# shenyunhang/APE

Hardware: NVIDIA H100
Metric: images_per_sec (higher is better)
Workload: dtype f16

## Files before the change

### ape_b200/csrc/gemm_tc.cu

```cuda
#include <stdlib.h>

#include <type_traits>

#include "common.cuh"
#include "tc.cuh"

namespace ape {
namespace {

constexpr int BM = 128, BK = 64, WG_K = 16;
constexpr int kConsumerWarps = 8;
constexpr int kThreads = 32 * kConsumerWarps + 32;

enum Act { ACT_NONE = 0, ACT_RELU = 1, ACT_GELU = 2, ACT_SWIGLU = 3, ACT_CLAMP = 4 };
enum Res { RES_NONE = 0, RES_F32 = 1, RES_16 = 2 };

template <bool OUT32, int ACT, int RES, bool LN = false, bool ROPE = false, bool STATS = false>
struct Epi {
  static constexpr bool out32 = OUT32, ln = LN, rope = ROPE, stats = STATS;
  static constexpr int act = ACT, res = RES;
};

struct GemmParams {
  void *C;
  const float *bias;
  const void *residual;
  long long ldc, ldr;
  int M, N, K;
  int m_blocks, n_blocks, k_blocks;
  int band;
  int vec_out;
  int fast;
  const float *rope_cos, *rope_sin;
  const int *rope_pos;
  int rope_cols, rope_npos;
  const float *ln_part;
  const float *ln_colsum;
  int ln_nparts;
  float ln_inv_c, ln_eps;
  float *stats_out;
  int stats_nslab;
  int conv;
  int conv_tw, conv_th, conv_tiles_x, conv_tiles_img, conv_cblks, conv_W, conv_H;
  long long *trace;
  int argmax_col_base;
};

__device__ __forceinline__ void trace_stamp(const GemmParams &p, int slot) {
  if (p.trace != nullptr) p.trace[(size_t)blockIdx.x * 8 + slot] = clock64();
}

template <int BN, int STAGES>
struct alignas(1024) GemmSmem {
  uint8_t a[STAGES][BM * BK * 2];
  uint8_t b[STAGES][BN * BK * 2];
  uint64_t full[STAGES], empty[STAGES];
};

template <int ACT>
__device__ __forceinline__ float act1(float v) {
  if constexpr (ACT == ACT_RELU) return fmaxf(v, 0.f);
  if constexpr (ACT == ACT_GELU) return 0.5f * v * (1.f + erff(v * 0.70710678118654752f));
  if constexpr (ACT == ACT_CLAMP) return fminf(fmaxf(v, -50000.f), 50000.f);
  return v;
}

template <bool VEC>
__device__ __forceinline__ float2 ld_pair(const float *p, int n, bool ok1) {
  if constexpr (VEC) return __ldg(reinterpret_cast<const float2 *>(p + n));
  return make_float2(__ldg(p + n), ok1 ? __ldg(p + n + 1) : 0.f);
}
template <bool VEC, typename T>
__device__ __forceinline__ float2 ld_res_pair(const T *p, bool ok1) {
  if constexpr (VEC) return Elem<T>::load2(p);
  return make_float2(Elem<T>::load1(p), ok1 ? Elem<T>::load1(p + 1) : 0.f);
}

__device__ __forceinline__ size_t out_row_offset(const GemmParams &p, int m) {
  if (!p.conv) return (size_t)m * p.ldc;
  const int m_blk = m / BM, r = m - m_blk * BM;
  const int img = m_blk / p.conv_tiles_img, t = m_blk - img * p.conv_tiles_img;
  const int ty = t / p.conv_tiles_x, tx = t - ty * p.conv_tiles_x;
  const int x = tx * p.conv_tw + r % p.conv_tw, y = ty * p.conv_th + r / p.conv_tw;
  return (((size_t)img * p.conv_H + y) * p.conv_W + x) * p.ldc;
}

template <typename TO>
__device__ __forceinline__ void store_pair(TO *dst, float v0, float v1, bool ok1, bool vec) {
  if (vec && ok1) {
    if constexpr (sizeof(TO) == 4) {
      *reinterpret_cast<float2 *>(dst) = make_float2(v0, v1);
    } else if constexpr (std::is_same<TO, __half>::value) {
      *reinterpret_cast<__half2 *>(dst) = __floats2half2_rn(v0, v1);
    } else {
      *reinterpret_cast<__nv_bfloat162 *>(dst) = __floats2bfloat162_rn(v0, v1);
    }
  } else {
    dst[0] = Elem<TO>::from_f(v0);
    if (ok1) dst[1] = Elem<TO>::from_f(v1);
  }
}

template <class E, typename TI, int BN, bool FULL>
__device__ __forceinline__ void epilogue(const GemmParams &p, const float *acc, int m_blk, int n_blk, int wg, int lane) {
  using TO = std::conditional_t<E::out32, float, TI>;
  constexpr bool swiglu = E::act == ACT_SWIGLU;
  const int warp4 = (threadIdx.x >> 5) & 3, tq = lane & 3;
  const int c_base = n_blk * BN + 2 * tq;
  TO *C = reinterpret_cast<TO *>(p.C);
#pragma unroll
  for (int h = 0; h < 2; ++h) {
    const int m = m_blk * BM + wg * 64 + warp4 * 16 + (lane >> 2) + 8 * h;
    const bool row_ok = FULL || m < p.M;
    const int mr = row_ok ? m : p.M - 1;
    float ln_rstd = 1.f, ln_shift = 0.f;
    if constexpr (E::ln) {
      const float2 *pp = reinterpret_cast<const float2 *>(p.ln_part) + (size_t)mr * p.ln_nparts;
      float sum = 0.f, sq = 0.f;
      for (int i = 0; i < p.ln_nparts; ++i) {
        const float2 t = __ldg(pp + i);
        sum += t.x;
        sq += t.y;
      }
      const float mean = sum * p.ln_inv_c;
      ln_rstd = rsqrtf(fmaxf(sq * p.ln_inv_c - mean * mean, 0.f) + p.ln_eps);
      ln_shift = ln_rstd * mean;
    }
    int rope_row = 0;
    if constexpr (E::rope) rope_row = (p.rope_pos ? __ldg(p.rope_pos + mr) : mr % p.rope_npos) * 64;
    TO *crow = C + out_row_offset(p, mr);
    const float *res32 = reinterpret_cast<const float *>(p.residual) + (size_t)mr * p.ldr;
    const TI *res16 = reinterpret_cast<const TI *>(p.residual) + (size_t)mr * p.ldr;
    float st_sum = 0.f, st_sq = 0.f;
#pragma unroll
    for (int j = 0; j < BN / 8; ++j) {
      const int n = c_base + 8 * j;
      const bool ok0 = FULL || n < p.N, ok1 = FULL || n + 1 < p.N;
      float v0 = acc[4 * j + 2 * h], v1 = acc[4 * j + 2 * h + 1];
      if (ok0) {
        if constexpr (E::ln) {
          const float2 cs = ld_pair<FULL>(p.ln_colsum, n, ok1);
          v0 = fmaf(ln_rstd, v0, -ln_shift * cs.x);
          if (ok1) v1 = fmaf(ln_rstd, v1, -ln_shift * cs.y);
        }
        if (p.bias != nullptr) {
          const float2 b = ld_pair<FULL && !E::ln>(p.bias, n, ok1);
          v0 += b.x;
          if (ok1) v1 += b.y;
        }
      }
      if constexpr (swiglu) {
        const float o = v0 / (1.f + __expf(-v0)) * v1;
        const TO ot = Elem<TO>::from_f(o);
        if (ok0 && row_ok) crow[n / 2] = ot;
        if constexpr (E::stats) {
          const float f = ok0 ? Elem<TO>::to_f(ot) : 0.f;
          st_sum += f;
          st_sq = fmaf(f, f, st_sq);
          if ((j & 15) == 15) {
            st_sum += __shfl_xor_sync(0xffffffffu, st_sum, 1);
            st_sq += __shfl_xor_sync(0xffffffffu, st_sq, 1);
            st_sum += __shfl_xor_sync(0xffffffffu, st_sum, 2);
            st_sq += __shfl_xor_sync(0xffffffffu, st_sq, 2);
            const int slab_idx = (n_blk * BN + 8 * (j - 15)) / 128;
            if (tq == 0 && row_ok && slab_idx < p.stats_nslab)
              *reinterpret_cast<float2 *>(p.stats_out + ((size_t)m * p.stats_nslab + slab_idx) * 2) = make_float2(st_sum, st_sq);
            st_sum = 0.f;
            st_sq = 0.f;
          }
        }
        continue;
      } else {
        if constexpr (E::rope) {
          if (n < p.rope_cols) {
            const float2 c = __ldg(reinterpret_cast<const float2 *>(p.rope_cos + rope_row + (n & 63)));
            const float2 s = __ldg(reinterpret_cast<const float2 *>(p.rope_sin + rope_row + (n & 63)));
            const float t0 = v0, t1 = v1;
            v0 = t0 * c.x - t1 * s.x;
            v1 = t1 * c.y + t0 * s.y;
          }
        }
        v0 = act1<E::act>(v0);
        v1 = act1<E::act>(v1);
        if constexpr (E::res != RES_NONE) {
          if (ok0) {
            const float2 r = E::res == RES_F32 ? ld_res_pair<FULL>(res32 + n, ok1) : ld_res_pair<FULL>(res16 + n, ok1);
            v0 += r.x;
            if (ok1) v1 += r.y;
          }
        }
        if (ok0 && row_ok) store_pair<TO>(crow + n, v0, v1, ok1, FULL || p.vec_out);
      }
    }
  }
}

struct EpiArgmax {
  static constexpr bool out32 = true, ln = false, rope = false, stats = false;
  static constexpr int act = ACT_NONE, res = RES_NONE;
};
template <class E>
constexpr bool kArgmax = std::is_same<E, EpiArgmax>::value;

template <int BN>
__device__ __forceinline__ void argmax_epilogue(const GemmParams &p, const float *acc, int m_blk, int n_blk, int wg, int lane) {
  const int warp4 = (threadIdx.x >> 5) & 3, tq = lane & 3;
  const int c_base = n_blk * BN + 2 * tq;
  unsigned long long *keys = reinterpret_cast<unsigned long long *>(p.C);
#pragma unroll
  for (int h = 0; h < 2; ++h) {
    const int m = m_blk * BM + wg * 64 + warp4 * 16 + (lane >> 2) + 8 * h;
    float best = -INFINITY;
    int col = -1;
#pragma unroll
    for (int j = 0; j < BN / 8; ++j) {
      const int n = c_base + 8 * j;
      const float v0 = acc[4 * j + 2 * h], v1 = acc[4 * j + 2 * h + 1];
      if (n < p.N && (col < 0 || v0 > best)) { best = v0; col = n; }
      if (n + 1 < p.N && v1 > best) { best = v1; col = n + 1; }
    }
#pragma unroll
    for (int s = 1; s <= 2; s <<= 1) {
      const float ob = __shfl_xor_sync(0xffffffffu, best, s);
      const int oc = __shfl_xor_sync(0xffffffffu, col, s);
      if (oc >= 0 && (col < 0 || ob > best || (ob == best && oc < col))) { best = ob; col = oc; }
    }
    if (tq == 0 && col >= 0 && m < p.M) atomicMax(keys + m, argmax_key(best, col + p.argmax_col_base));
  }
}

template <int BN, int STAGES, int CL, typename TI, class E>
__global__ void __launch_bounds__(kThreads, 1)
gemm_tc_kernel(const __grid_constant__ CUtensorMap map_a, const __grid_constant__ CUtensorMap map_b, const GemmParams p) {
  extern __shared__ uint8_t smem_raw[];
  pdl_launch_dependents();
  if (threadIdx.x == 0) trace_stamp(p, 0);
  using Smem = GemmSmem<BN, STAGES>;
  Smem &s = *reinterpret_cast<Smem *>((reinterpret_cast<uintptr_t>(smem_raw) + 1023) & ~uintptr_t(1023));
  constexpr uint32_t STAGE_BYTES = (BM + BN) * BK * 2;

  const int warp = threadIdx.x / 32, lane = threadIdx.x % 32;
  const int rank = CL > 1 ? (int)tc::cluster_ctarank() : 0;
  const int m_groups = (p.m_blocks + CL - 1) / CL;
  const int num_tiles = m_groups * p.n_blocks;
  const int first = blockIdx.x / CL, stride = gridDim.x / CL;
  auto tile_at = [&](int t, int &m_blk, int &n_blk) -> bool {
    const int tile = first + t * stride;
    if (tile >= num_tiles) return false;
    const int per_band = p.band * p.n_blocks;
    const int band = tile / per_band, r = tile - band * per_band;
    const int rows = min(p.band, m_groups - band * p.band);
    n_blk = r / rows;
    m_blk = (band * p.band + r - n_blk * rows) * CL + rank;
    return true;
  };

  if (warp == kConsumerWarps && lane == 0) {
    tc::prefetch_tensormap(&map_a);
    tc::prefetch_tensormap(&map_b);
#pragma unroll
    for (int i = 0; i < STAGES; ++i) {
      tc::mbar_init(&s.full[i], 1);
      tc::mbar_init(&s.empty[i], kConsumerWarps * CL);
    }
    tc::fence_mbar_init();
  }
  __syncthreads();
  if (CL > 1) tc::cluster_sync_all();
  pdl_wait();
  if (threadIdx.x == 0) trace_stamp(p, 1);

  if (warp == kConsumerWarps) {
    if (lane == 0) {
      uint32_t stage = 0, phase = 0;
      int m_blk, n_blk;
      for (int t = 0; tile_at(t, m_blk, n_blk); ++t) {
        for (int kb = 0; kb < p.k_blocks; ++kb) {
          tc::mbar_wait(&s.empty[stage], phase ^ 1);
          tc::mbar_expect_tx(&s.full[stage], STAGE_BYTES);
          if (p.conv) {
            const int img = m_blk / p.conv_tiles_img, tt = m_blk - img * p.conv_tiles_img;
            const int ty = tt / p.conv_tiles_x, tx = tt - ty * p.conv_tiles_x;
            const int tap = kb / p.conv_cblks, cb = kb - tap * p.conv_cblks;
            tc::tma_load_4d(s.a[stage], &map_a, &s.full[stage], cb * BK, tx * p.conv_tw + tap % 3 - 1, ty * p.conv_th + tap / 3 - 1, img);
          } else {
            tc::tma_load_2d(s.a[stage], &map_a, &s.full[stage], kb * BK, m_blk * BM);
          }
          if (CL == 1) {
            tc::tma_load_2d(s.b[stage], &map_b, &s.full[stage], kb * BK, n_blk * BN);
          } else {
            constexpr int HALF_ROWS = BN / CL;
            tc::tma_load_2d_multicast(s.b[stage] + rank * HALF_ROWS * BK * 2, &map_b, &s.full[stage], kb * BK,
                                      n_blk * BN + rank * HALF_ROWS, (uint16_t)((1u << CL) - 1));
          }
          if (++stage == STAGES) { stage = 0; phase ^= 1; }
        }
      }
    }
    __syncwarp();
  } else {
    const int wg = warp / 4;
    float acc[BN / 2];
#pragma unroll
    for (int i = 0; i < BN / 2; ++i) acc[i] = 0.f;
    auto release = [&](uint32_t st) {
      if (lane == 0) {
        tc::mbar_arrive(&s.empty[st]);
        if (CL > 1) tc::mbar_arrive_cluster(tc::mapa_u32(&s.empty[st], (uint32_t)(rank ^ 1)));
      }
    };
    uint32_t stage = 0, phase = 0;
    int m_blk, n_blk;
    for (int t = 0; tile_at(t, m_blk, n_blk); ++t) {
      uint32_t prev = 0;
      for (int kb = 0; kb < p.k_blocks; ++kb) {
        tc::mbar_wait(&s.full[stage], phase);
        if (kb == 0 && t == 0 && threadIdx.x == 0) trace_stamp(p, 2);
        const uint64_t da = tc::make_smem_desc_sw128(tc::smem_u32(s.a[stage] + wg * 64 * BK * 2));
        const uint64_t db = tc::make_smem_desc_sw128(tc::smem_u32(s.b[stage]));
        tc::fence_regs<BN / 2>(acc);
        tc::wgmma_fence();
#pragma unroll
        for (int k = 0; k < BK / WG_K; ++k)
          tc::Wgmma<BN, TI>::template ss<0>(acc, da + 2 * k, db + 2 * k, (kb | k) != 0);
        tc::wgmma_commit();
        tc::fence_regs<BN / 2>(acc);
        if (kb > 0) {
          tc::wgmma_wait<1>();
          release(prev);
        }
        prev = stage;
        if (++stage == STAGES) { stage = 0; phase ^= 1; }
      }
      tc::wgmma_wait<0>();
      tc::fence_regs<BN / 2>(acc);
      release(prev);
      if (threadIdx.x == 0) {
        trace_stamp(p, 3);
        if (t == 0) trace_stamp(p, 4);
        trace_stamp(p, 5);
      }
      if constexpr (kArgmax<E>) argmax_epilogue<BN>(p, acc, m_blk, n_blk, wg, lane);
      else if (!E::rope && p.fast && (m_blk + 1) * BM <= p.M && (n_blk + 1) * BN <= p.N) epilogue<E, TI, BN, true>(p, acc, m_blk, n_blk, wg, lane);
      else epilogue<E, TI, BN, false>(p, acc, m_blk, n_blk, wg, lane);
    }
    if (threadIdx.x == 0) trace_stamp(p, 6);
  }
  __syncthreads();
  if (CL > 1) tc::cluster_sync_all();
  if (threadIdx.x == 0) trace_stamp(p, 7);
}

constexpr int kPpThreads = 32 * kConsumerWarps + 128;
constexpr int kOrderBar = 1;

template <typename TI, class E>
__global__ void __launch_bounds__(kPpThreads, 1)
gemm_pp_kernel(const __grid_constant__ CUtensorMap map_a, const __grid_constant__ CUtensorMap map_b, const GemmParams p) {
  constexpr int BN = 128, STAGES = 6;
  extern __shared__ uint8_t smem_raw[];
  pdl_launch_dependents();
  if (threadIdx.x == 0) trace_stamp(p, 0);
  using Smem = GemmSmem<BN, STAGES>;
  Smem &s = *reinterpret_cast<Smem *>((reinterpret_cast<uintptr_t>(smem_raw) + 1023) & ~uintptr_t(1023));
  constexpr uint32_t STAGE_BYTES = (BM + BN) * BK * 2;

  const int warp = threadIdx.x / 32, lane = threadIdx.x % 32;
  const int num_tiles = p.m_blocks * p.n_blocks;
  auto tile_at = [&](int t, int &m_blk, int &n_blk) -> bool {
    const int tile = blockIdx.x + t * gridDim.x;
    if (tile >= num_tiles) return false;
    const int per_band = p.band * p.n_blocks;
    const int band = tile / per_band, r = tile - band * per_band;
    const int rows = min(p.band, p.m_blocks - band * p.band);
    n_blk = r / rows;
    m_blk = band * p.band + r - n_blk * rows;
    return true;
  };

  if (warp == kConsumerWarps && lane == 0) {
    tc::prefetch_tensormap(&map_a);
    tc::prefetch_tensormap(&map_b);
#pragma unroll
    for (int i = 0; i < STAGES; ++i) {
      tc::mbar_init(&s.full[i], 1);
      tc::mbar_init(&s.empty[i], 4);
    }
    tc::fence_mbar_init();
  }
  __syncthreads();
  pdl_wait();
  if (threadIdx.x == 0) trace_stamp(p, 1);

  if (warp >= kConsumerWarps) {
    tc::setmaxnreg_dec<40>();
    if (warp == kConsumerWarps && lane == 0) {
      uint32_t stage = 0, phase = 0;
      int m_blk, n_blk;
      for (int t = 0; tile_at(t, m_blk, n_blk); ++t) {
        for (int kb = 0; kb < p.k_blocks; ++kb) {
          tc::mbar_wait(&s.empty[stage], phase ^ 1);
          tc::mbar_expect_tx(&s.full[stage], STAGE_BYTES);
          tc::tma_load_2d(s.a[stage], &map_a, &s.full[stage], kb * BK, m_blk * BM);
          tc::tma_load_2d(s.b[stage], &map_b, &s.full[stage], kb * BK, n_blk * BN);
          if (++stage == STAGES) { stage = 0; phase ^= 1; }
        }
      }
    }
    __syncwarp();
  } else {
    tc::setmaxnreg_inc<232>();
    const int wg = warp / 4;
    float acc[BN];
#pragma unroll
    for (int i = 0; i < BN; ++i) acc[i] = 0.f;
    auto release = [&](uint32_t st) {
      if (lane == 0) tc::mbar_arrive(&s.empty[st]);
    };
    int m_blk, n_blk;
    for (int t = wg; tile_at(t, m_blk, n_blk); t += 2) {
      if (t > 0) tc::named_bar_sync(kOrderBar + wg, 256);
      const uint32_t g0 = (uint32_t)t * p.k_blocks;
      uint32_t stage = g0 % STAGES, phase = (g0 / STAGES) & 1, prev = 0;
      for (int kb = 0; kb < p.k_blocks; ++kb) {
        tc::mbar_wait(&s.full[stage], phase);
        if (kb == 0 && t == 0 && threadIdx.x == 0) trace_stamp(p, 2);
        const uint64_t da = tc::make_smem_desc_sw128(tc::smem_u32(s.a[stage]));
        const uint64_t da_hi = tc::make_smem_desc_sw128(tc::smem_u32(s.a[stage] + 64 * BK * 2));
        const uint64_t db = tc::make_smem_desc_sw128(tc::smem_u32(s.b[stage]));
        tc::fence_regs<BN>(acc);
        tc::wgmma_fence();
#pragma unroll
        for (int k = 0; k < BK / WG_K; ++k) {
          tc::Wgmma<BN, TI>::template ss<0>(acc, da + 2 * k, db + 2 * k, (kb | k) != 0);
          tc::Wgmma<BN, TI>::template ss<0>(acc + 64, da_hi + 2 * k, db + 2 * k, (kb | k) != 0);
        }
        tc::wgmma_commit();
        tc::fence_regs<BN>(acc);
        if (kb > 0) {
          tc::wgmma_wait<1>();
          release(prev);
        }
        prev = stage;
        if (++stage == STAGES) { stage = 0; phase ^= 1; }
      }
      int m_nx, n_nx;
      if (tile_at(t + 1, m_nx, n_nx)) tc::named_bar_arrive(kOrderBar + (wg ^ 1), 256);
      tc::wgmma_wait<0>();
      tc::fence_regs<BN>(acc);
      release(prev);
      if (threadIdx.x == 0) {
        trace_stamp(p, 3);
        if (t == 0) trace_stamp(p, 4);
        trace_stamp(p, 5);
      }
      if constexpr (kArgmax<E>) {
        argmax_epilogue<BN>(p, acc, m_blk, n_blk, 0, lane);
        argmax_epilogue<BN>(p, acc + 64, m_blk, n_blk, 1, lane);
      } else if (!E::rope && p.fast && (m_blk + 1) * BM <= p.M && (n_blk + 1) * BN <= p.N) {
        epilogue<E, TI, BN, true>(p, acc, m_blk, n_blk, 0, lane);
        epilogue<E, TI, BN, true>(p, acc + 64, m_blk, n_blk, 1, lane);
      } else {
        epilogue<E, TI, BN, false>(p, acc, m_blk, n_blk, 0, lane);
        epilogue<E, TI, BN, false>(p, acc + 64, m_blk, n_blk, 1, lane);
      }
    }
    if (threadIdx.x == 0) trace_stamp(p, 6);
  }
  __syncthreads();
  if (threadIdx.x == 0) trace_stamp(p, 7);
}

constexpr int BK8 = 128;

template <typename TO, class E>
__global__ void __launch_bounds__(kThreads, 1)
gemm_fp8_kernel(const __grid_constant__ CUtensorMap map_a, const __grid_constant__ CUtensorMap map_b, const GemmParams p,
                const float *__restrict__ a_scale, const float *__restrict__ w_scale) {
  constexpr int BN = 128, STAGES = 6;
  extern __shared__ uint8_t smem_raw[];
  pdl_launch_dependents();
  using Smem = GemmSmem<BN, STAGES>;
  Smem &s = *reinterpret_cast<Smem *>((reinterpret_cast<uintptr_t>(smem_raw) + 1023) & ~uintptr_t(1023));
  constexpr uint32_t STAGE_BYTES = (BM + BN) * BK8;

  const int warp = threadIdx.x / 32, lane = threadIdx.x % 32;
  const int num_tiles = p.m_blocks * p.n_blocks;
  auto tile_at = [&](int t, int &m_blk, int &n_blk) -> bool {
    const int tile = blockIdx.x + t * gridDim.x;
    if (tile >= num_tiles) return false;
    const int per_band = p.band * p.n_blocks;
    const int band = tile / per_band, r = tile - band * per_band;
    const int rows = min(p.band, p.m_blocks - band * p.band);
    n_blk = r / rows;
    m_blk = band * p.band + r - n_blk * rows;
    return true;
  };

  if (warp == kConsumerWarps && lane == 0) {
    tc::prefetch_tensormap(&map_a);
    tc::prefetch_tensormap(&map_b);
#pragma unroll
    for (int i = 0; i < STAGES; ++i) {
      tc::mbar_init(&s.full[i], 1);
      tc::mbar_init(&s.empty[i], kConsumerWarps);
    }
    tc::fence_mbar_init();
  }
  __syncthreads();
  pdl_wait();

  if (warp == kConsumerWarps) {
    if (lane == 0) {
      uint32_t stage = 0, phase = 0;
      int m_blk, n_blk;
      for (int t = 0; tile_at(t, m_blk, n_blk); ++t) {
        for (int kb = 0; kb < p.k_blocks; ++kb) {
          tc::mbar_wait(&s.empty[stage], phase ^ 1);
          tc::mbar_expect_tx(&s.full[stage], STAGE_BYTES);
          tc::tma_load_2d(s.a[stage], &map_a, &s.full[stage], kb * BK8, m_blk * BM);
          tc::tma_load_2d(s.b[stage], &map_b, &s.full[stage], kb * BK8, n_blk * BN);
          if (++stage == STAGES) { stage = 0; phase ^= 1; }
        }
      }
    }
    __syncwarp();
  } else {
    const int wg = warp / 4, warp4 = warp & 3, tq = lane & 3;
    float acc[BN / 2], part[BN / 2];
    uint32_t stage = 0, phase = 0;
    int m_blk, n_blk;
    for (int t = 0; tile_at(t, m_blk, n_blk); ++t) {
#pragma unroll
      for (int i = 0; i < BN / 2; ++i) acc[i] = 0.f;
      for (int kb = 0; kb < p.k_blocks; ++kb) {
        tc::mbar_wait(&s.full[stage], phase);
        const uint64_t da = tc::make_smem_desc_sw128(tc::smem_u32(s.a[stage] + wg * 64 * BK8));
        const uint64_t db = tc::make_smem_desc_sw128(tc::smem_u32(s.b[stage]));
        tc::fence_regs<BN / 2>(part);
        tc::wgmma_fence();
#pragma unroll
        for (int k = 0; k < BK8 / 32; ++k)
          tc::Wgmma<BN, __nv_fp8_e4m3>::template ss<0>(part, da + 2 * k, db + 2 * k, k != 0);
        tc::wgmma_commit();
        tc::wgmma_wait<0>();
        tc::fence_regs<BN / 2>(part);
        if (lane == 0) tc::mbar_arrive(&s.empty[stage]);
#pragma unroll
        for (int i = 0; i < BN / 2; ++i) acc[i] += part[i];
        if (++stage == STAGES) { stage = 0; phase ^= 1; }
      }
      const int m0 = m_blk * BM + wg * 64 + warp4 * 16 + (lane >> 2);
      const float sa0 = __ldg(a_scale + min(m0, p.M - 1)), sa1 = __ldg(a_scale + min(m0 + 8, p.M - 1));
#pragma unroll
      for (int j = 0; j < BN / 8; ++j) {
        const int n = n_blk * BN + 8 * j + 2 * tq;
        const float sw0 = n < p.N ? __ldg(w_scale + n) : 0.f, sw1 = n + 1 < p.N ? __ldg(w_scale + n + 1) : 0.f;
        acc[4 * j] = acc[4 * j] * sa0 * sw0;
        acc[4 * j + 1] = acc[4 * j + 1] * sa0 * sw1;
        acc[4 * j + 2] = acc[4 * j + 2] * sa1 * sw0;
        acc[4 * j + 3] = acc[4 * j + 3] * sa1 * sw1;
      }
      if (p.fast && (m_blk + 1) * BM <= p.M && (n_blk + 1) * BN <= p.N) epilogue<E, TO, BN, true>(p, acc, m_blk, n_blk, wg, lane);
      else epilogue<E, TO, BN, false>(p, acc, m_blk, n_blk, wg, lane);
    }
  }
  __syncthreads();
}

typedef CUresult (*EncodeTiledFn)(CUtensorMap *, CUtensorMapDataType, cuuint32_t, void *, const cuuint64_t *,
                                  const cuuint64_t *, const cuuint32_t *, const cuuint32_t *, CUtensorMapInterleave,
                                  CUtensorMapSwizzle, CUtensorMapL2promotion, CUtensorMapFloatOOBfill);

EncodeTiledFn get_encoder() {
  static EncodeTiledFn fn = nullptr;
  if (fn == nullptr) {
    void *ptr = nullptr;
    cudaDriverEntryPointQueryResult qres;
    if (cudaGetDriverEntryPoint("cuTensorMapEncodeTiled", &ptr, cudaEnableDefault, &qres) == cudaSuccess &&
        qres == cudaDriverEntryPointSuccess)
      fn = reinterpret_cast<EncodeTiledFn>(ptr);
  }
  return fn;
}

int make_map(CUtensorMap *map, const void *base, int dtype, long long rows, long long K, long long ld, int box_rows,
             int box_cols = BK) {
  EncodeTiledFn enc = get_encoder();
  if (!enc) return fail(APE_ERR_UNSUPPORTED, "gemm: cuTensorMapEncodeTiled not available from the driver");
  cuuint64_t dims[2] = {(cuuint64_t)K, (cuuint64_t)rows};
  cuuint64_t strides[1] = {(cuuint64_t)ld * (dtype == APE_DTYPE_F32 ? 4 : dtype == APE_DTYPE_E4M3 ? 1 : 2)};
  cuuint32_t box[2] = {(cuuint32_t)box_cols, (cuuint32_t)box_rows};
  cuuint32_t estr[2] = {1, 1};
  CUresult r = enc(map, dtype == APE_DTYPE_F32 ? CU_TENSOR_MAP_DATA_TYPE_FLOAT32
                        : dtype == APE_DTYPE_E4M3 ? CU_TENSOR_MAP_DATA_TYPE_UINT8
                        : dtype == APE_DTYPE_F16 ? CU_TENSOR_MAP_DATA_TYPE_FLOAT16 : CU_TENSOR_MAP_DATA_TYPE_BFLOAT16, 2,
                   const_cast<void *>(base), dims, strides, box, estr, CU_TENSOR_MAP_INTERLEAVE_NONE,
                   CU_TENSOR_MAP_SWIZZLE_128B, CU_TENSOR_MAP_L2_PROMOTION_L2_256B, CU_TENSOR_MAP_FLOAT_OOB_FILL_NONE);
  if (r != CUDA_SUCCESS) return fail(APE_ERR_INVALID_ARG, "gemm: cuTensorMapEncodeTiled failed (%d)", (int)r);
  return APE_OK;
}

int num_sms() {
  static int n = 0;
  if (n == 0) {
    int dev = 0;
    cudaGetDevice(&dev);
    cudaDeviceGetAttribute(&n, cudaDevAttrMultiProcessorCount, dev);
    if (n <= 0) n = 132;
  }
  return n;
}

template <int BN, int STAGES, int CL, typename TI, class E, bool PP = false>
int launch_gemm(const CUtensorMap &ma, const CUtensorMap &mb, GemmParams &p, cudaStream_t st) {
  static_assert(!PP || (BN == 128 && STAGES == 6 && CL == 1), "gemm_pp_kernel is BN = 128, 6 stages, single CTA");
  using Smem = GemmSmem<BN, STAGES>;
  const size_t smem = sizeof(Smem) + 1024;
  auto k = PP ? gemm_pp_kernel<TI, E> : gemm_tc_kernel<BN, STAGES, CL, TI, E>;
  static bool attr_set = false;
  if (!attr_set) {
    cudaError_t e = cudaFuncSetAttribute(k, cudaFuncAttributeMaxDynamicSharedMemorySize, (int)smem);
    if (e != cudaSuccess) return fail((int)e, "gemm: cudaFuncSetAttribute(smem=%zu): %s", smem, cudaGetErrorString(e));
    attr_set = true;
  }
  p.n_blocks = (p.N + BN - 1) / BN;
  const int m_groups = (p.m_blocks + CL - 1) / CL;
  const int groups = m_groups * p.n_blocks;
  const int max_clusters = num_sms() / CL;
  const int clusters = groups < max_clusters ? groups : max_clusters;
  p.band = std::min(m_groups, (clusters + p.n_blocks - 1) / p.n_blocks);
  cudaLaunchConfig_t cfg{};
  cfg.gridDim = dim3((unsigned)(clusters * CL));
  cfg.blockDim = dim3(PP ? kPpThreads : kThreads);
  cfg.dynamicSmemBytes = smem;
  cfg.stream = st;
  cudaLaunchAttribute attr[2];
  attr[0].id = cudaLaunchAttributeClusterDimension;
  attr[0].val.clusterDim.x = CL;
  attr[0].val.clusterDim.y = 1;
  attr[0].val.clusterDim.z = 1;
  attr[1].id = cudaLaunchAttributeProgrammaticStreamSerialization;
  attr[1].val.programmaticStreamSerializationAllowed = pdl_enabled() ? 1 : 0;
  cfg.attrs = attr;
  cfg.numAttrs = 2;
  cudaError_t e = cudaLaunchKernelEx(&cfg, k, ma, mb, p);
  if (e != cudaSuccess) return fail((int)e, "gemm_tc_kernel launch: %s", cudaGetErrorString(e));
  return check_launch("gemm_tc_kernel");
}

template <int CL, typename TI, class E>
int launch_bn(int bn, bool pp, const CUtensorMap &ma, const CUtensorMap &mb, GemmParams &p, cudaStream_t st) {
  if (bn == 256) return launch_gemm<256, 4, CL, TI, E>(ma, mb, p, st);
  if constexpr (CL == 1)
    if (pp) return launch_gemm<128, 6, 1, TI, E, true>(ma, mb, p, st);
  return launch_gemm<128, 6, CL, TI, E>(ma, mb, p, st);
}

struct EpiKey {
  bool out32;
  int act, res;
  bool ln, rope, stats;
};

#define APE_GEMM_EPILOGUES(X)                                                                                            \
  X(false, ACT_NONE, RES_NONE, false, false, false) X(false, ACT_RELU, RES_NONE, false, false, false)                   \
  X(false, ACT_GELU, RES_NONE, false, false, false) X(false, ACT_NONE, RES_F32, false, false, false)                    \
  X(false, ACT_NONE, RES_16, false, false, false) X(false, ACT_RELU, RES_16, false, false, false)                       \
  X(false, ACT_GELU, RES_16, false, false, false) X(false, ACT_SWIGLU, RES_NONE, false, false, false)                   \
  X(false, ACT_SWIGLU, RES_NONE, false, false, true) X(false, ACT_NONE, RES_NONE, false, true, false)                   \
  X(true, ACT_NONE, RES_NONE, false, false, false) X(true, ACT_RELU, RES_NONE, false, false, false)                     \
  X(true, ACT_GELU, RES_NONE, false, false, false) X(true, ACT_SWIGLU, RES_NONE, false, false, false)                   \
  X(true, ACT_CLAMP, RES_NONE, false, false, false) X(true, ACT_NONE, RES_F32, false, false, false)                     \
  X(true, ACT_NONE, RES_16, false, false, false) X(true, ACT_NONE, RES_F32, true, false, false)

template <int CL, typename TI>
int launch_epi(int bn, bool pp, const EpiKey &k, const CUtensorMap &ma, const CUtensorMap &mb, GemmParams &p, cudaStream_t st) {
#define APE_EPI_CASE(o, a, r, l, ro, s)                                                                                  \
  if (k.out32 == o && k.act == a && k.res == r && k.ln == l && k.rope == ro && k.stats == s)                           \
    return launch_bn<CL, TI, Epi<o, a, r, l, ro, s>>(bn, pp, ma, mb, p, st);
  APE_GEMM_EPILOGUES(APE_EPI_CASE)
#undef APE_EPI_CASE
  return fail(APE_ERR_UNSUPPORTED, "gemm: no kernel for the epilogue (fp32 out %d, act %d, residual %d, ln %d, rope %d, stats %d)",
              (int)k.out32, k.act, k.res, (int)k.ln, (int)k.rope, (int)k.stats);
}

int launch_any(int bn, bool cluster, bool pp, int in_dtype, const EpiKey &k, const CUtensorMap &ma, const CUtensorMap &mb,
               GemmParams &p, cudaStream_t st) {
  if (in_dtype == APE_DTYPE_BF16)
    return cluster ? launch_epi<2, __nv_bfloat16>(bn, false, k, ma, mb, p, st) : launch_epi<1, __nv_bfloat16>(bn, pp, k, ma, mb, p, st);
  return cluster ? launch_epi<2, __half>(bn, false, k, ma, mb, p, st) : launch_epi<1, __half>(bn, pp, k, ma, mb, p, st);
}

bool use_pingpong(int tiles) { return tiles >= 2 * num_sms(); }

template <typename TO, class E>
int launch_fp8(const CUtensorMap &ma, const CUtensorMap &mb, GemmParams &p, const float *a_scale, const float *w_scale,
               cudaStream_t st) {
  constexpr int BN = 128;
  const size_t smem = sizeof(GemmSmem<BN, 6>) + 1024;
  auto k = gemm_fp8_kernel<TO, E>;
  static bool attr_set = false;
  if (!attr_set) {
    cudaError_t e = cudaFuncSetAttribute(k, cudaFuncAttributeMaxDynamicSharedMemorySize, (int)smem);
    if (e != cudaSuccess) return fail((int)e, "gemm_e4m3: cudaFuncSetAttribute(smem=%zu): %s", smem, cudaGetErrorString(e));
    attr_set = true;
  }
  p.n_blocks = (p.N + BN - 1) / BN;
  const int tiles = p.m_blocks * p.n_blocks;
  const int ctas = std::min(tiles, num_sms());
  p.band = std::min(p.m_blocks, (ctas + p.n_blocks - 1) / p.n_blocks);
  APE_LAUNCH(k, ctas, kThreads, smem, st, ma, mb, p, a_scale, w_scale);
  return check_launch("gemm_fp8_kernel");
}

template <typename TO>
int launch_fp8_epi(int act, bool stats, const CUtensorMap &ma, const CUtensorMap &mb, GemmParams &p, const float *a_scale,
                   const float *w_scale, cudaStream_t st) {
  if (act == ACT_NONE && !stats) return launch_fp8<TO, Epi<false, ACT_NONE, RES_NONE>>(ma, mb, p, a_scale, w_scale, st);
  if (act == ACT_SWIGLU && !stats) return launch_fp8<TO, Epi<false, ACT_SWIGLU, RES_NONE>>(ma, mb, p, a_scale, w_scale, st);
  if (act == ACT_SWIGLU) return launch_fp8<TO, Epi<false, ACT_SWIGLU, RES_NONE, false, false, true>>(ma, mb, p, a_scale, w_scale, st);
  return fail(APE_ERR_UNSUPPORTED, "gemm_e4m3: no kernel for activation %d (none or swiglu only)", act);
}

}
}

using namespace ape;

struct RopeArgs {
  const float *cos, *sin;
  const int *pos;
  int cols, npos;
};

struct FuseArgs {
  const float *ln_part, *ln_colsum;
  int ln_nparts;
  float ln_inv_c, ln_eps;
  float *stats_out;
  int stats_nslab;
};

static long long *g_gemm_trace = nullptr;

extern "C" void ape_gemm_set_trace(long long *device_buffer) { g_gemm_trace = device_buffer; }

static int gemm_impl(const void *A, int64_t lda, const void *W, int64_t ldw, void *C, int64_t ldc,
                     const float *bias, const void *residual, int64_t ldr, int res_dtype, int M, int N, int K, int in_dtype,
                     int out_dtype, int act, int tile_n, const RopeArgs *rope, void *stream, const FuseArgs *fuse = nullptr) {
  if (residual && res_dtype != APE_DTYPE_F32 && res_dtype != APE_DTYPE_F16 && res_dtype != APE_DTYPE_BF16)
    return fail(APE_ERR_INVALID_ARG, "gemm: bad res_dtype %d", res_dtype);
  if (in_dtype != APE_DTYPE_F16 && in_dtype != APE_DTYPE_BF16)
    return fail(APE_ERR_INVALID_ARG, "gemm: operands must be fp16 or bf16 (got dtype %d)", in_dtype);
  if (out_dtype != APE_DTYPE_F32 && out_dtype != APE_DTYPE_F16 && out_dtype != APE_DTYPE_BF16)
    return fail(APE_ERR_INVALID_ARG, "gemm: bad out_dtype %d", out_dtype);
  if (act < 0 || act > ACT_CLAMP) return fail(APE_ERR_INVALID_ARG, "gemm: bad activation %d", act);
  if (M < 0 || N <= 0 || K <= 0) return fail(APE_ERR_INVALID_ARG, "gemm: bad sizes M=%d N=%d K=%d", M, N, K);
  if (M == 0) return APE_OK;
  if (!A || !W || !C) return fail(APE_ERR_NULL_PTR, "gemm: null pointer argument");
  if ((lda * 2) % 16 || (ldw * 2) % 16 || (reinterpret_cast<uintptr_t>(A) & 15) || (reinterpret_cast<uintptr_t>(W) & 15))
    return fail(APE_ERR_INVALID_ARG, "gemm: A/W base and row pitch must be 16-byte aligned (TMA)");
  if (lda < K || ldw < K) return fail(APE_ERR_INVALID_ARG, "gemm: row pitch smaller than K");
  if (act == ACT_SWIGLU && ((N & 1) || residual)) return fail(APE_ERR_INVALID_ARG, "gemm: swiglu needs even N, no residual");
  const int bn = (tile_n & 0xfff) > 0 ? (tile_n & 0xfff) : 128;
  if (bn != 128 && bn != 256) return fail(APE_ERR_INVALID_ARG, "gemm: tile_n must be 128 or 256");
  if (tile_n & 0x2000) return fail(APE_ERR_UNSUPPORTED, "gemm: tile_n flag 0x2000 (CTA-pair MMA) is not available on sm_90a");
  cudaStream_t st = reinterpret_cast<cudaStream_t>(stream);
  const bool force_pp = (tile_n & 0x8000) != 0, force_coop = (tile_n & 0x10000) != 0;
  if (force_pp && (force_coop || bn != 128 || (tile_n & 0x4000)))
    return fail(APE_ERR_INVALID_ARG, "gemm: tile_n flag 0x8000 (ping-pong) needs tile width 128, no cluster and no 0x10000");
  const int m_blocks = (M + BM - 1) / BM;
  const bool cluster = m_blocks >= 2 && !force_pp && (tile_n & 0x1000) == 0 && ((tile_n & 0x4000) != 0 || K >= 2048);
  const bool pp = !cluster && bn == 128 && !force_coop && (force_pp || use_pingpong(m_blocks * ((N + bn - 1) / bn)));
  CUtensorMap ma, mb;
  if (int rc = make_map(&ma, A, in_dtype, M, K, lda, BM)) return rc;
  if (int rc = make_map(&mb, W, in_dtype, N, K, ldw, cluster ? bn / 2 : bn)) return rc;
  GemmParams p{};
  p.C = C; p.bias = bias; p.residual = residual; p.ldc = ldc; p.ldr = ldr;
  p.M = M; p.N = N; p.K = K;
  p.m_blocks = m_blocks;
  p.k_blocks = (K + BK - 1) / BK;
  p.trace = g_gemm_trace;
  const int oe = out_dtype == APE_DTYPE_F32 ? 4 : 2;
  if (oe == 2 && out_dtype != in_dtype)
    return fail(APE_ERR_UNSUPPORTED, "gemm: a 16-bit output must have the operand dtype (out %d, operands %d)", out_dtype, in_dtype);
  if (residual && res_dtype != APE_DTYPE_F32 && res_dtype != in_dtype)
    return fail(APE_ERR_UNSUPPORTED, "gemm: a 16-bit residual must have the operand dtype (residual %d, operands %d)", res_dtype, in_dtype);
  const auto pairs = [](const void *ptr, long long ld, int esize) {
    return (ld % 2) == 0 && (reinterpret_cast<uintptr_t>(ptr) % (2 * esize)) == 0;
  };
  p.vec_out = pairs(C, ldc, oe);
  p.fast = p.vec_out && (!residual || pairs(residual, ldr, res_dtype == APE_DTYPE_F32 ? 4 : 2)) &&
           reinterpret_cast<uintptr_t>(bias) % 8 == 0 && (!fuse || reinterpret_cast<uintptr_t>(fuse->ln_colsum) % 8 == 0);
  EpiKey key{oe == 4, act, !residual ? RES_NONE : res_dtype == APE_DTYPE_F32 ? RES_F32 : RES_16, false, rope != nullptr, false};
  const int n_out = act == ACT_SWIGLU ? N / 2 : N;
  if (fuse) {
    if (fuse->ln_part) {
      if (out_dtype != APE_DTYPE_F32 || !fuse->ln_colsum || fuse->ln_nparts <= 0 || act == ACT_SWIGLU)
        return fail(APE_ERR_INVALID_ARG, "gemm+ln: needs an fp32 output, column sums and partial statistics");
      p.ln_part = fuse->ln_part; p.ln_colsum = fuse->ln_colsum; p.ln_nparts = fuse->ln_nparts;
      p.ln_inv_c = fuse->ln_inv_c; p.ln_eps = fuse->ln_eps;
      key.ln = true;
    }
    if (fuse->stats_out) {
      if (oe != 2 || act != ACT_SWIGLU || fuse->stats_nslab != (n_out + 63) / 64)
        return fail(APE_ERR_INVALID_ARG, "gemm+stats: needs the SwiGLU epilogue with a 16-bit output and stats_nslab = ceil(N/2/64)");
      p.stats_out = fuse->stats_out; p.stats_nslab = fuse->stats_nslab;
      key.stats = true;
    }
  }
  if (rope) {
    if (oe != 2 || act != ACT_NONE || rope->cols % 64 != 0 || rope->cols > N || rope->npos <= 0 || !rope->cos || !rope->sin)
      return fail(APE_ERR_INVALID_ARG, "gemm+rope: needs a 16-bit output, no activation, rope_cols a multiple of 64 <= N");
    p.rope_cos = rope->cos; p.rope_sin = rope->sin; p.rope_pos = rope->pos; p.rope_cols = rope->cols; p.rope_npos = rope->npos;
  }
  return launch_any(bn, cluster, pp, in_dtype, key, ma, mb, p, st);
}

extern "C" int ape_gemm_tn(const void *A, int64_t lda, const void *W, int64_t ldw, void *C, int64_t ldc,
                           const float *bias, const void *residual, int64_t ldr, int M, int N, int K, int in_dtype,
                           int out_dtype, int act, int tile_n, void *stream) {
  return gemm_impl(A, lda, W, ldw, C, ldc, bias, residual, ldr, out_dtype, M, N, K, in_dtype, out_dtype, act, tile_n, nullptr,
                   stream);
}

extern "C" int ape_gemm_tn_ex(const void *A, int64_t lda, const void *W, int64_t ldw, void *C, int64_t ldc,
                              const float *bias, const void *residual, int64_t ldr, int res_dtype, int M, int N, int K,
                              int in_dtype, int out_dtype, int act, int tile_n, void *stream) {
  return gemm_impl(A, lda, W, ldw, C, ldc, bias, residual, ldr, res_dtype, M, N, K, in_dtype, out_dtype, act, tile_n, nullptr,
                   stream);
}

extern "C" int ape_gemm_tn_fused(const void *A, int64_t lda, const void *W, int64_t ldw, void *C, int64_t ldc, const float *bias,
                                 const void *residual, int64_t ldr, int res_dtype, int M, int N, int K, int in_dtype, int out_dtype,
                                 int act, int tile_n, const float *ln_part, int ln_nparts, const float *ln_colsum, float ln_inv_c,
                                 float ln_eps, float *stats_out, int stats_nslab, void *stream) {
  FuseArgs f{ln_part, ln_colsum, ln_nparts, ln_inv_c, ln_eps, stats_out, stats_nslab};
  return gemm_impl(A, lda, W, ldw, C, ldc, bias, residual, ldr, res_dtype, M, N, K, in_dtype, out_dtype, act, tile_n, nullptr,
                   stream, &f);
}

static int make_map_nhwc(CUtensorMap *map, const void *base, int dtype, int B, int H, int W, int C, int bw, int bh) {
  EncodeTiledFn enc = get_encoder();
  if (!enc) return fail(APE_ERR_UNSUPPORTED, "conv: cuTensorMapEncodeTiled not available from the driver");
  cuuint64_t dims[4] = {(cuuint64_t)C, (cuuint64_t)W, (cuuint64_t)H, (cuuint64_t)B};
  cuuint64_t strides[3] = {(cuuint64_t)C * 2, (cuuint64_t)W * C * 2, (cuuint64_t)H * W * C * 2};
  cuuint32_t box[4] = {64, (cuuint32_t)bw, (cuuint32_t)bh, 1};
  cuuint32_t estr[4] = {1, 1, 1, 1};
  CUresult r = enc(map, dtype == APE_DTYPE_F16 ? CU_TENSOR_MAP_DATA_TYPE_FLOAT16 : CU_TENSOR_MAP_DATA_TYPE_BFLOAT16, 4,
                   const_cast<void *>(base), dims, strides, box, estr, CU_TENSOR_MAP_INTERLEAVE_NONE,
                   CU_TENSOR_MAP_SWIZZLE_128B, CU_TENSOR_MAP_L2_PROMOTION_L2_256B, CU_TENSOR_MAP_FLOAT_OOB_FILL_NONE);
  if (r != CUDA_SUCCESS) return fail(APE_ERR_INVALID_ARG, "conv: cuTensorMapEncodeTiled failed (%d)", (int)r);
  return APE_OK;
}

extern "C" int ape_conv3x3_nhwc(const void *x, const void *w, void *y, const float *bias, int B, int H, int W, int Cin, int Cout,
                                int dtype, int act, void *stream) {
  if (dtype != APE_DTYPE_F16 && dtype != APE_DTYPE_BF16) return fail(APE_ERR_INVALID_ARG, "conv3x3: fp16 / bf16 only");
  if (B <= 0 || H <= 0 || W <= 0 || Cin <= 0 || Cout <= 0) return fail(APE_ERR_INVALID_ARG, "conv3x3: bad sizes");
  if (Cin % 64 || Cout % 8) return fail(APE_ERR_UNSUPPORTED, "conv3x3: Cin must be a multiple of 64 and Cout of 8 (got %d, %d)", Cin, Cout);
  if (act != ACT_NONE && act != ACT_RELU && act != ACT_GELU) return fail(APE_ERR_INVALID_ARG, "conv3x3: activation %d", act);
  int tw = 128;
  while (tw > 8 && W % tw) tw >>= 1;
  const int th = 128 / tw;
  if (W % tw || H % th) return fail(APE_ERR_UNSUPPORTED, "conv3x3: %dx%d image is not a whole number of %dx%d pixel tiles", H, W, th, tw);
  if (!x || !w || !y) return fail(APE_ERR_NULL_PTR, "conv3x3: null pointer argument");
  if ((reinterpret_cast<uintptr_t>(x) | reinterpret_cast<uintptr_t>(w) | reinterpret_cast<uintptr_t>(y)) & 15)
    return fail(APE_ERR_INVALID_ARG, "conv3x3: tensors must be 16-byte aligned");
  const int K = 9 * Cin, M = B * H * W, N = Cout;
  const int bn = 128;
  const int m_blocks = M / BM;
  const bool cluster = m_blocks >= 2 && m_blocks % 2 == 0;
  CUtensorMap ma, mb;
  if (int rc = make_map_nhwc(&ma, x, dtype, B, H, W, Cin, tw, th)) return rc;
  if (int rc = make_map(&mb, w, dtype, N, K, K, cluster ? bn / 2 : bn)) return rc;
  GemmParams p{};
  p.C = y; p.bias = bias; p.ldc = N; p.M = M; p.N = N; p.K = K;
  p.m_blocks = m_blocks;
  p.k_blocks = K / BK;
  p.vec_out = 1;
  p.fast = reinterpret_cast<uintptr_t>(bias) % 8 == 0;
  p.conv = 1; p.conv_tw = tw; p.conv_th = th; p.conv_tiles_x = W / tw; p.conv_tiles_img = (W / tw) * (H / th); p.conv_cblks = Cin / 64;
  p.conv_W = W; p.conv_H = H;
  const EpiKey key{false, act, RES_NONE, false, false, false};
  return launch_any(bn, cluster, false, dtype, key, ma, mb, p, reinterpret_cast<cudaStream_t>(stream));
}

extern "C" int ape_gemm_tn_argmax(const void *A, int64_t lda, const void *W, int64_t ldw, uint64_t *keys, int M, int N, int K,
                                  int col_base, int in_dtype, void *stream) {
  if (in_dtype != APE_DTYPE_F16 && in_dtype != APE_DTYPE_BF16)
    return fail(APE_ERR_INVALID_ARG, "gemm_argmax: operands must be fp16 or bf16 (got dtype %d)", in_dtype);
  if (M < 0 || N <= 0 || K <= 0 || col_base < 0 || (long long)col_base + N > 0x7fffffffLL)
    return fail(APE_ERR_INVALID_ARG, "gemm_argmax: bad sizes M=%d N=%d K=%d col_base=%d", M, N, K, col_base);
  if (M == 0) return APE_OK;
  if (!A || !W || !keys) return fail(APE_ERR_NULL_PTR, "gemm_argmax: null pointer argument");
  if ((lda * 2) % 16 || (ldw * 2) % 16 || (reinterpret_cast<uintptr_t>(A) & 15) || (reinterpret_cast<uintptr_t>(W) & 15))
    return fail(APE_ERR_INVALID_ARG, "gemm_argmax: A/W base and row pitch must be 16-byte aligned (TMA)");
  if (lda < K || ldw < K) return fail(APE_ERR_INVALID_ARG, "gemm_argmax: row pitch smaller than K");
  if (reinterpret_cast<uintptr_t>(keys) & 7) return fail(APE_ERR_INVALID_ARG, "gemm_argmax: keys must be 8-byte aligned");
  constexpr int bn = 128;
  CUtensorMap ma, mb;
  if (int rc = make_map(&ma, A, in_dtype, M, K, lda, BM)) return rc;
  if (int rc = make_map(&mb, W, in_dtype, N, K, ldw, bn)) return rc;
  GemmParams p{};
  p.C = keys; p.M = M; p.N = N; p.K = K;
  p.m_blocks = (M + BM - 1) / BM;
  p.k_blocks = (K + BK - 1) / BK;
  p.trace = g_gemm_trace;
  p.argmax_col_base = col_base;
  cudaStream_t st = reinterpret_cast<cudaStream_t>(stream);
  if (use_pingpong(p.m_blocks * ((N + bn - 1) / bn))) {
    if (in_dtype == APE_DTYPE_BF16) return launch_gemm<bn, 6, 1, __nv_bfloat16, EpiArgmax, true>(ma, mb, p, st);
    return launch_gemm<bn, 6, 1, __half, EpiArgmax, true>(ma, mb, p, st);
  }
  if (in_dtype == APE_DTYPE_BF16) return launch_gemm<bn, 6, 1, __nv_bfloat16, EpiArgmax>(ma, mb, p, st);
  return launch_gemm<bn, 6, 1, __half, EpiArgmax>(ma, mb, p, st);
}

extern "C" int ape_gemm_tn_rope(const void *A, int64_t lda, const void *W, int64_t ldw, void *C, int64_t ldc,
                                const float *bias, int M, int N, int K, int in_dtype, int out_dtype, const float *cos_table,
                                const float *sin_table, const int *pos_map, int npos, int head_dim, int rope_cols,
                                int tile_n, void *stream) {
  if (head_dim != 64) return fail(APE_ERR_UNSUPPORTED, "gemm+rope: head_dim %d (only 64)", head_dim);
  if ((reinterpret_cast<uintptr_t>(cos_table) | reinterpret_cast<uintptr_t>(sin_table)) & 15)
    return fail(APE_ERR_INVALID_ARG, "gemm+rope: cos / sin tables must be 16-byte aligned");
  RopeArgs r{cos_table, sin_table, pos_map, rope_cols, npos};
  return gemm_impl(A, lda, W, ldw, C, ldc, bias, nullptr, 0, out_dtype, M, N, K, in_dtype, out_dtype, ACT_NONE, tile_n, &r, stream);
}

extern "C" int ape_gemm_tn_e4m3(const void *A, int64_t lda, const void *W, int64_t ldw, const float *a_scale,
                                const float *w_scale, void *C, int64_t ldc, const float *bias, int M, int N, int K, int out_dtype,
                                int act, float *stats_out, int stats_nslab, void *stream) {
  if (out_dtype != APE_DTYPE_F16 && out_dtype != APE_DTYPE_BF16)
    return fail(APE_ERR_UNSUPPORTED, "gemm_e4m3: output must be fp16 or bf16 (got dtype %d)", out_dtype);
  if (act != ACT_NONE && act != ACT_SWIGLU)
    return fail(APE_ERR_UNSUPPORTED, "gemm_e4m3: no kernel for activation %d (none or swiglu only)", act);
  if (M < 0 || N <= 0 || K <= 0) return fail(APE_ERR_INVALID_ARG, "gemm_e4m3: bad sizes M=%d N=%d K=%d", M, N, K);
  if (K % 16) return fail(APE_ERR_INVALID_ARG, "gemm_e4m3: K must be a multiple of 16 (got %d)", K);
  if (M == 0) return APE_OK;
  if (!A || !W || !C) return fail(APE_ERR_NULL_PTR, "gemm_e4m3: null pointer argument");
  if (!a_scale || !w_scale) return fail(APE_ERR_NULL_PTR, "gemm_e4m3: null scale pointer (a_scale [M] and w_scale [N] are required)");
  if (lda % 16 || ldw % 16 || (reinterpret_cast<uintptr_t>(A) & 15) || (reinterpret_cast<uintptr_t>(W) & 15))
    return fail(APE_ERR_INVALID_ARG, "gemm_e4m3: A/W base and row pitch must be 16-byte aligned (TMA)");
  if (lda < K || ldw < K) return fail(APE_ERR_INVALID_ARG, "gemm_e4m3: row pitch smaller than K");
  if ((reinterpret_cast<uintptr_t>(a_scale) | reinterpret_cast<uintptr_t>(w_scale)) & 3)
    return fail(APE_ERR_INVALID_ARG, "gemm_e4m3: scales must be 4-byte aligned fp32");
  if (act == ACT_SWIGLU && (N & 1)) return fail(APE_ERR_INVALID_ARG, "gemm_e4m3: swiglu needs even N");
  const int n_out = act == ACT_SWIGLU ? N / 2 : N;
  if (stats_out && (act != ACT_SWIGLU || stats_nslab != (n_out + 63) / 64))
    return fail(APE_ERR_INVALID_ARG, "gemm_e4m3+stats: needs the SwiGLU epilogue and stats_nslab = ceil(N/2/64)");
  CUtensorMap ma, mb;
  if (int rc = make_map(&ma, A, APE_DTYPE_E4M3, M, K, lda, BM, BK8)) return rc;
  if (int rc = make_map(&mb, W, APE_DTYPE_E4M3, N, K, ldw, 128, BK8)) return rc;
  GemmParams p{};
  p.C = C; p.bias = bias; p.ldc = ldc;
  p.M = M; p.N = N; p.K = K;
  p.m_blocks = (M + BM - 1) / BM;
  p.k_blocks = (K + BK8 - 1) / BK8;
  p.vec_out = (ldc % 2) == 0 && (reinterpret_cast<uintptr_t>(C) % 4) == 0;
  p.fast = p.vec_out && reinterpret_cast<uintptr_t>(bias) % 8 == 0;
  p.stats_out = stats_out;
  p.stats_nslab = stats_out ? stats_nslab : 0;
  cudaStream_t st = reinterpret_cast<cudaStream_t>(stream);
  if (out_dtype == APE_DTYPE_BF16) return launch_fp8_epi<__nv_bfloat16>(act, stats_out != nullptr, ma, mb, p, a_scale, w_scale, st);
  return launch_fp8_epi<__half>(act, stats_out != nullptr, ma, mb, p, a_scale, w_scale, st);
}
```

Baseline: 40.03.

## Use 256-wide N tiles for large GEMMs with producer/consumer register split

Adds a heuristic that picks a 256-column tile instead of the 2-CTA cluster path for large N and K (N>=1024, K>=2048). The cooperative kernel gets a full producer warpgroup so it can use setmaxnreg to move registers from producers to consumers, which hold the doubled accumulator. The epilogue is split into two 128-column halves so existing epilogue code is reused. The aim is more operand reuse per CTA and fewer B loads, at the cost of register pressure, larger smem stages, and coarser tile counts that can leave SMs idle with wave quantization.

Result: faster. 42.51 (median of 6 runs) (+6.2%).

```diff
diff --git a/ape_b200/csrc/gemm_tc.cu b/ape_b200/csrc/gemm_tc.cu
--- a/ape_b200/csrc/gemm_tc.cu
+++ b/ape_b200/csrc/gemm_tc.cu
@@ -10,7 +10,8 @@
 
 constexpr int BM = 128, BK = 64, WG_K = 16;
 constexpr int kConsumerWarps = 8;
-constexpr int kThreads = 32 * kConsumerWarps + 32;
+constexpr int kThreads = 32 * kConsumerWarps + 128;
+constexpr int kProducerRegs = 40, kConsumerRegs = 232;
 
 enum Act { ACT_NONE = 0, ACT_RELU = 1, ACT_GELU = 2, ACT_SWIGLU = 3, ACT_CLAMP = 4 };
 enum Res { RES_NONE = 0, RES_F32 = 1, RES_16 = 2 };
@@ -270,8 +271,9 @@
   pdl_wait();
   if (threadIdx.x == 0) trace_stamp(p, 1);
 
-  if (warp == kConsumerWarps) {
-    if (lane == 0) {
+  if (warp >= kConsumerWarps) {
+    tc::setmaxnreg_dec<kProducerRegs>();
+    if (warp == kConsumerWarps && lane == 0) {
       uint32_t stage = 0, phase = 0;
       int m_blk, n_blk;
       for (int t = 0; tile_at(t, m_blk, n_blk); ++t) {
@@ -299,6 +301,7 @@
     }
     __syncwarp();
   } else {
+    tc::setmaxnreg_inc<kConsumerRegs>();
     const int wg = warp / 4;
     float acc[BN / 2];
 #pragma unroll
@@ -340,9 +343,16 @@
         if (t == 0) trace_stamp(p, 4);
         trace_stamp(p, 5);
       }
-      if constexpr (kArgmax<E>) argmax_epilogue<BN>(p, acc, m_blk, n_blk, wg, lane);
-      else if (!E::rope && p.fast && (m_blk + 1) * BM <= p.M && (n_blk + 1) * BN <= p.N) epilogue<E, TI, BN, true>(p, acc, m_blk, n_blk, wg, lane);
-      else epilogue<E, TI, BN, false>(p, acc, m_blk, n_blk, wg, lane);
+      if constexpr (kArgmax<E>) {
+        argmax_epilogue<BN>(p, acc, m_blk, n_blk, wg, lane);
+      } else {
+#pragma unroll
+        for (int h = 0; h < BN / 128; ++h) {
+          const int nb = n_blk * (BN / 128) + h;
+          if (!E::rope && p.fast && (m_blk + 1) * BM <= p.M && (nb + 1) * 128 <= p.N) epilogue<E, TI, 128, true>(p, acc + 64 * h, m_blk, nb, wg, lane);
+          else epilogue<E, TI, 128, false>(p, acc + 64 * h, m_blk, nb, wg, lane);
+        }
+      }
     }
     if (threadIdx.x == 0) trace_stamp(p, 6);
   }
@@ -351,11 +361,10 @@
   if (threadIdx.x == 0) trace_stamp(p, 7);
 }
 
-constexpr int kPpThreads = 32 * kConsumerWarps + 128;
 constexpr int kOrderBar = 1;
 
 template <typename TI, class E>
-__global__ void __launch_bounds__(kPpThreads, 1)
+__global__ void __launch_bounds__(kThreads, 1)
 gemm_pp_kernel(const __grid_constant__ CUtensorMap map_a, const __grid_constant__ CUtensorMap map_b, const GemmParams p) {
   constexpr int BN = 128, STAGES = 6;
   extern __shared__ uint8_t smem_raw[];
@@ -393,7 +402,7 @@
   if (threadIdx.x == 0) trace_stamp(p, 1);
 
   if (warp >= kConsumerWarps) {
-    tc::setmaxnreg_dec<40>();
+    tc::setmaxnreg_dec<kProducerRegs>();
     if (warp == kConsumerWarps && lane == 0) {
       uint32_t stage = 0, phase = 0;
       int m_blk, n_blk;
@@ -409,7 +418,7 @@
     }
     __syncwarp();
   } else {
-    tc::setmaxnreg_inc<232>();
+    tc::setmaxnreg_inc<kConsumerRegs>();
     const int wg = warp / 4;
     float acc[BN];
 #pragma unroll
@@ -472,9 +481,10 @@
 }
 
 constexpr int BK8 = 128;
+constexpr int kFp8Threads = 32 * kConsumerWarps + 32;
 
 template <typename TO, class E>
-__global__ void __launch_bounds__(kThreads, 1)
+__global__ void __launch_bounds__(kFp8Threads, 1)
 gemm_fp8_kernel(const __grid_constant__ CUtensorMap map_a, const __grid_constant__ CUtensorMap map_b, const GemmParams p,
                 const float *__restrict__ a_scale, const float *__restrict__ w_scale) {
   constexpr int BN = 128, STAGES = 6;
@@ -632,7 +642,7 @@
   p.band = std::min(m_groups, (clusters + p.n_blocks - 1) / p.n_blocks);
   cudaLaunchConfig_t cfg{};
   cfg.gridDim = dim3((unsigned)(clusters * CL));
-  cfg.blockDim = dim3(PP ? kPpThreads : kThreads);
+  cfg.blockDim = dim3(kThreads);
   cfg.dynamicSmemBytes = smem;
   cfg.stream = st;
   cudaLaunchAttribute attr[2];
@@ -694,6 +704,8 @@
 
 bool use_pingpong(int tiles) { return tiles >= 2 * num_sms(); }
 
+bool use_wide(int N, int K) { return N >= 1024 && K >= 2048; }
+
 template <typename TO, class E>
 int launch_fp8(const CUtensorMap &ma, const CUtensorMap &mb, GemmParams &p, const float *a_scale, const float *w_scale,
                cudaStream_t st) {
@@ -710,7 +722,7 @@
   const int tiles = p.m_blocks * p.n_blocks;
   const int ctas = std::min(tiles, num_sms());
   p.band = std::min(p.m_blocks, (ctas + p.n_blocks - 1) / p.n_blocks);
-  APE_LAUNCH(k, ctas, kThreads, smem, st, ma, mb, p, a_scale, w_scale);
+  APE_LAUNCH(k, ctas, kFp8Threads, smem, st, ma, mb, p, a_scale, w_scale);
   return check_launch("gemm_fp8_kernel");
 }
 
@@ -763,15 +775,16 @@
     return fail(APE_ERR_INVALID_ARG, "gemm: A/W base and row pitch must be 16-byte aligned (TMA)");
   if (lda < K || ldw < K) return fail(APE_ERR_INVALID_ARG, "gemm: row pitch smaller than K");
   if (act == ACT_SWIGLU && ((N & 1) || residual)) return fail(APE_ERR_INVALID_ARG, "gemm: swiglu needs even N, no residual");
-  const int bn = (tile_n & 0xfff) > 0 ? (tile_n & 0xfff) : 128;
+  const bool force_pp = (tile_n & 0x8000) != 0, force_coop = (tile_n & 0x10000) != 0;
+  const int m_blocks = (M + BM - 1) / BM;
+  const bool wide = (tile_n & 0xfff) == 0 && !force_pp && !force_coop && use_wide(N, K);
+  const int bn = (tile_n & 0xfff) > 0 ? (tile_n & 0xfff) : wide ? 256 : 128;
   if (bn != 128 && bn != 256) return fail(APE_ERR_INVALID_ARG, "gemm: tile_n must be 128 or 256");
   if (tile_n & 0x2000) return fail(APE_ERR_UNSUPPORTED, "gemm: tile_n flag 0x2000 (CTA-pair MMA) is not available on sm_90a");
   cudaStream_t st = reinterpret_cast<cudaStream_t>(stream);
-  const bool force_pp = (tile_n & 0x8000) != 0, force_coop = (tile_n & 0x10000) != 0;
   if (force_pp && (force_coop || bn != 128 || (tile_n & 0x4000)))
     return fail(APE_ERR_INVALID_ARG, "gemm: tile_n flag 0x8000 (ping-pong) needs tile width 128, no cluster and no 0x10000");
-  const int m_blocks = (M + BM - 1) / BM;
-  const bool cluster = m_blocks >= 2 && !force_pp && (tile_n & 0x1000) == 0 && ((tile_n & 0x4000) != 0 || K >= 2048);
+  const bool cluster = m_blocks >= 2 && !force_pp && (tile_n & 0x1000) == 0 && ((tile_n & 0x4000) != 0 || (!wide && K >= 2048));
   const bool pp = !cluster && bn == 128 && !force_coop && (force_pp || use_pingpong(m_blocks * ((N + bn - 1) / bn)));
   CUtensorMap ma, mb;
   if (int rc = make_map(&ma, A, in_dtype, M, K, lda, BM)) return rc;
```
